# ksahlin/BESST

Hardware: AMD Instinct MI355X
Metric: read-pairs/sec into scaffold graph; edge-set match + gap MAE vs CPU ref (higher is better)
Workload: dtype int32/int64 (fp64 for read_len truncation); 1 GPU; C3: 100000 contigs / 200000000 read-pairs, one rf library with 22 % PE contamination, 400000000 records resident in HBM (1 copy cycled); records_per_gpu=400000000, edge_rows=263235, parallelism=single GPU, generator=besst_amd.synth.simulate_library_device (torch ops on the GPU, seeded), 1.5 s

## Files before the change

### besst_amd/csrc/classify.hip

```cpp
#include <stdarg.h>
#include <stdio.h>
#include <stdlib.h>

#include <atomic>
#include <type_traits>

#include "common.h"

namespace besst {

namespace {

constexpr uint32_t kNoSlot = 0xffffffffu;

constexpr uint32_t EV_COV = 1u, EV_FISHY = 2u, EV_NONUNIQ = 4u, EV_REACH = 8u,
                   EV_DOUBLE = 32u, EV_MAPQ0 = 64u, EV_CASEA = 128u, EV_FIRSTMIN = 256u;

enum : int { kSpecGeneric = 0, kSpecFr = 1, kSpecRf = 2 };

__device__ __forceinline__ uint32_t ins_thr_u32(const ClassifyArgs& a) {
    return a.ins_thr_int <= 0 ? 0u : (uint32_t)a.ins_thr_int;
}

struct Eval {
// ... 1299 lines not shown
        a.has_any = last_idx >= 0 ? 1 : 0;
        a.l1 = last_idx >= 0 ? s_l1[last_idx] : 0;
        a.l2 = last_idx >= 0 ? s_l2[last_idx] : 0;
        a.head_present = s_first[0] > 0 ? 1 : 0;
        a.f1 = s_first[1]; a.f2 = s_first[2]; a.head_info = (uint32_t)s_first[3];
        int tot = 0, tot_runs = 0;
        for (int w = 0; w < 16; ++w) { tot += s_sum[w]; tot_runs += s_sum_runs[w]; }
        a.total = (uint32_t)tot;
        a.runs = (uint32_t)tot_runs;
        agg[blockIdx.x] = a;
    }
}

template <bool kRuns>
__global__ __launch_bounds__(1024) void stitch_kernel(SummView summ, uint32_t nblocks, int32_t* carry, int detect,
                                                      uint32_t* __restrict__ offsets,
                                                      uint32_t* __restrict__ skip_slot,
                                                      uint32_t* n_out,
                                                      unsigned long long* counters,
                                                      const int32_t* __restrict__ tails, int rank,
                                                      int32_t* __restrict__ slice_info,
                                                      const StitchAgg* __restrict__ agg,
                                                      const int32_t* __restrict__ carry_in, uint32_t span,
                                                      uint32_t* __restrict__ run_offsets) {
    __shared__ int32_t s_l1[1024 * kStitchRounds], s_l2[1024 * kStitchRounds];
    __shared__ int s_any;
    __shared__ int s_head_block;
    __shared__ int32_t s_head[4];
    __shared__ int s_tab[64];
    __shared__ int s_total;
    using acc_t = typename std::conditional<kRuns, long long, int>::type;
    auto pack_counts = [](uint32_t tuples, uint32_t runs) -> acc_t {
        if (kRuns) return (acc_t)((long long)tuples | ((long long)runs << 32));
        return (acc_t)tuples;
    };
    __shared__ acc_t s_tab64[64];
    __shared__ acc_t s_total64;
    __shared__ int32_t s_carry[2];
    __shared__ acc_t s_base;
    __shared__ int s_redc[16][7];
    const int t = threadIdx.x, lane = t & 63, wave = t >> 6;
    const bool last_span = blockIdx.x == gridDim.x - 1;
    if (t == 0) {
        int32_t p1 = agg ? carry_in[0] : carry[0], p2 = agg ? carry_in[1] : carry[1];
        if (tails)
            for (int j = 0; j < rank; ++j)
                if (tails[j * 4]) { p1 = tails[j * 4 + 1]; p2 = tails[j * 4 + 2]; }
        int any = 0;
        acc_t base = 0;
        for (uint32_t j = 0; j < blockIdx.x; ++j) {
            const StitchAgg a = agg[j];
            acc_t tot = (acc_t)a.total;
            if (kRuns) tot = (acc_t)((long long)a.total | ((long long)a.runs << 32));
            if (a.head_present && !(slice_info && !any)) {
                const CEDelta d = create_edge(a.f1, a.f2, p1, p2, a.head_info & 1u, a.head_info & 2u, a.head_info & 4u,
                                              detect != 0);
                if ((a.head_info & 8u) && !d.keep) tot -= 1ll + (a.runs ? 1ll << 32 : 0ll);
            }
            base += tot;
            if (a.has_any) { p1 = a.l1; p2 = a.l2; any = 1; }
        }
        s_carry[0] = p1; s_carry[1] = p2; s_base = base;
        s_any = any; s_head_block = -1;
    }
    __syncthreads();
// ... 317 lines not shown
    __syncthreads();
    if (threadIdx.x == 0) {
        atomicAdd(&counts[0], (unsigned long long)(s_c[0] + s_c[1] + s_c[2] + s_c[3]));
        atomicAdd(&counts[1], (unsigned long long)(s_m[0] + s_m[1] + s_m[2] + s_m[3]));
    }
}

__global__ void resolve_carry_kernel(const int32_t* __restrict__ tails, int rank, int32_t* __restrict__ carry) {
    if (threadIdx.x != 0) return;
    for (int j = 0; j < rank; ++j)
        if (tails[j * 4]) { carry[0] = tails[j * 4 + 1]; carry[1] = tails[j * 4 + 2]; }
}

}

namespace {
std::atomic<int> g_last_form{-1};
}
int classify_last_form() { return g_last_form.load(); }

bool classify_can_group_runs(const ClassifyArgs& a) {
    static const int knob = [] { const char* e = getenv("BESST_LOOP_RUNS"); return e ? atoi(e) : 1; }();
    return knob != 0 && a.record_path == 1 && a.n > 0;
}

int launch_classify_scan(hipStream_t s, const ClassifyArgs& a, int64_t* aligned, besst_counters* counters,
                         void* ws, size_t ws_bytes, bool group_runs) {
    if (a.n <= 0) return BESST_OK;
    BESST_REQUIRE(a.n < (int64_t)1 << 32, "classify: more than 2^32-1 records in one call");
    const ClsWorkspace w = carve(ws, a.n);
    BESST_REQUIRE(ws != nullptr && ws_bytes >= w.total, "classify: workspace too small");
    const uint32_t nblocks = (uint32_t)((a.n + kClsTile - 1) / kClsTile);
    const uint32_t stream_blocks = (uint32_t)((a.n + kStreamTile - 1) / kStreamTile);
    BESST_REQUIRE(!group_runs || classify_can_group_runs(a), "classify: this record loop cannot group runs");
    if (a.record_path == 1) {
        if (group_runs) BESST_HIP_TRY(hipMemsetAsync(w.run_status, 0, 4, s));
        ProfScope ps(s, kProfFusedWave);
        auto* al = reinterpret_cast<unsigned long long*>(aligned);
        const bool side = a.cs_off && a.mate_bits && a.tid_bits;
        g_last_form.store(side ? 3 : a.mate_bits ? (a.tid_bits ? 2 : 1) : 0);
        if (side) {
            const uint32_t full = (uint32_t)(a.n / kClsTile);
            const char* const spec_env = getenv("BESST_LOOP_SPEC");
            const bool spec = !(spec_env && atoi(spec_env) == 0) && a.read_len_int >= 0 && a.extend_paths != 0 && a.no_score == 0 && a.detect_dup != 0;
            const int form = spec ? (a.rf != 0 ? kSpecRf : kSpecFr) : kSpecGeneric;
#define BESST_LAUNCH_LEAN(RUNS, SPEC)                                                                                   \
// ... 277 lines not shown
int launch_classify_emit(hipStream_t s, int64_t n, int detect_dup, int32_t* carry, uint64_t* keys,
                         uint64_t* payload, uint32_t* n_out, besst_counters* counters, void* ws,
                         size_t ws_bytes, const uint8_t* cls8, int32_t n_contigs, int64_t* aligned,
                         const int32_t* tails, int rank, int32_t* slice_info, PresortSpec* presort) {
    PresortSpec pre{};
    if (presort && presort->table) {
        pre = *presort;
        BESST_REQUIRE(pre.rows > 0 && (pre.rows & (pre.rows - 1)) == 0 && pre.shift >= 0 && pre.shift <= 47, "classify: bad presort description");
        if (!pre.in_record_loop) BESST_HIP_TRY(hipMemsetAsync(pre.table, 0, (size_t)pre.rows * 512 * sizeof(uint32_t), s));
    }
    if (n <= 0) {
        BESST_HIP_TRY(hipMemsetAsync(n_out, 0, sizeof(uint32_t), s));
        if (slice_info) BESST_HIP_TRY(hipMemsetAsync(slice_info, 0, 8 * sizeof(int32_t), s));
        if (presort) presort->segmented = 0;
        return BESST_OK;
    }
    const ClsWorkspace w = carve(ws, n);
    BESST_REQUIRE(ws != nullptr && ws_bytes >= w.total, "classify: workspace too small");
    const uint32_t nblocks = (uint32_t)((n + kClsTile - 1) / kClsTile);
    auto* ctr = reinterpret_cast<unsigned long long*>(counters);
    const bool grouped = pre.table && pre.in_record_loop == 3;
    BESST_REQUIRE(!grouped || (pre.segmented && !slice_info && !tails), "classify: grouped runs need the segmented hand-over");
    uint32_t* run_offsets = grouped ? w.run_offsets : nullptr;
    {
        ProfScope ps(s, kProfStitch);
        uint32_t span = kStitchSpan;
        if (const char* e = getenv("BESST_STITCH_SPAN")) {
            const long v = atol(e);
            if (v >= 1 && v < (long)kStitchSpan) span = (uint32_t)v;
        }
        const uint32_t spans = (nblocks + span - 1) / span;
        BESST_REQUIRE(spans <= w.agg_spans, "classify: too many stitch spans for the workspace");
        if (spans > 1) {
            int32_t* carry_in = reinterpret_cast<int32_t*>(w.agg + w.agg_spans);
            hipLaunchKernelGGL(stitch_spans_kernel, dim3(spans), dim3(1024), 0, s, w.summ, nblocks, span, detect_dup, carry,
                               w.agg, carry_in);
            if (run_offsets)
                hipLaunchKernelGGL(stitch_kernel<true>, dim3(spans), dim3(1024), 0, s, w.summ, nblocks, carry, detect_dup, w.offsets,
                                   w.skip, n_out, ctr, tails, rank, slice_info, w.agg, carry_in, span, run_offsets);
            else
                hipLaunchKernelGGL(stitch_kernel<false>, dim3(spans), dim3(1024), 0, s, w.summ, nblocks, carry, detect_dup, w.offsets,
                                   w.skip, n_out, ctr, tails, rank, slice_info, w.agg, carry_in, span, run_offsets);
        } else {
            if (run_offsets)
                hipLaunchKernelGGL(stitch_kernel<true>, dim3(1), dim3(1024), 0, s, w.summ, nblocks, carry, detect_dup, w.offsets,
                                   w.skip, n_out, ctr, tails, rank, slice_info, (const StitchAgg*)nullptr,
                                   (const int32_t*)nullptr, span, run_offsets);
            else
                hipLaunchKernelGGL(stitch_kernel<false>, dim3(1), dim3(1024), 0, s, w.summ, nblocks, carry, detect_dup, w.offsets,
                                   w.skip, n_out, ctr, tails, rank, slice_info, (const StitchAgg*)nullptr,
                                   (const int32_t*)nullptr, span, run_offsets);
        }
    }
    {
        PresortSpec in_compact = pre;
        const bool segmented = pre.table && pre.in_record_loop && pre.segmented && !slice_info && !tails;
        if (pre.table && pre.in_record_loop) {
            ProfScope ps(s, kProfFixup);
            hipLaunchKernelGGL(presort_fixup_kernel, dim3((nblocks + 255) / 256), dim3(256), 0, s, w.seg_keys, w.skip, nblocks, pre,
                               segmented ? cls8 : nullptr, n_contigs, reinterpret_cast<unsigned long long*>(aligned),
                               w.offsets, n_out, (segmented && !grouped) ? w.chunk_first : nullptr);
            in_compact.table = nullptr;
        }
        if (segmented) {
            presort->segmented = 1;
            presort->seg = SegSource{w.seg_keys, w.seg_payload, w.offsets, w.skip, nblocks, (uint32_t)kClsTile, payload, w.chunk_first,
                                     grouped ? w.run_offsets : nullptr, w.summ.p, w.summ.stride, w.run_status};
        } else {
            if (presort) presort->segmented = 0;
            ProfScope ps(s, kProfCompact);
            hipLaunchKernelGGL(compact_kernel, dim3(nblocks), dim3(256), 0, s, w.summ, w.offsets, w.skip, w.seg_keys,
                               w.seg_payload, keys, payload, cls8, n_contigs, reinterpret_cast<unsigned long long*>(aligned),
                               in_compact);
        }
    }
    BESST_HIP_TRY(hipGetLastError());
    return BESST_OK;
}

int launch_classify(hipStream_t s, const ClassifyArgs& a, int32_t* carry, int64_t* aligned, uint64_t* keys,
// ... 29 lines not shown
```

### besst_amd/csrc/common.h

```cpp
#pragma once

#include <hip/hip_runtime.h>
#include <stdint.h>

#include "../../include/besst_amd.h"
#include "bgzf_scan.h"

namespace besst {

void set_error(const char* fmt, ...);

#define BESST_HIP_TRY(expr)                                                                  \
    do {                                                                                     \
        hipError_t _e = (expr);                                                              \
        if (_e != hipSuccess) {                                                              \
            besst::set_error("%s failed: %s (%s:%d)", #expr, hipGetErrorString(_e), __FILE__, \
                             __LINE__);                                                      \
            return BESST_ERR_HIP;                                                            \
        }                                                                                    \
    } while (0)

#define BESST_REQUIRE(cond, msg)                 \
    do {                                         \
        if (!(cond)) {                           \
// ... 257 lines not shown
int launch_candidate_density(hipStream_t s, int64_t n, const int32_t* tid, const int32_t* mtid, int64_t sample_records,
                             unsigned long long* counts);
int launch_mate_bits(hipStream_t s, const int32_t* tid, const int32_t* mtid, int64_t lo, int64_t hi, int64_t n, uint8_t* bits,
                     uint8_t* tid_bits);
int launch_cand_offsets(hipStream_t s, int64_t n, int64_t n_refs, const int32_t* tid, const int32_t* mtid,
                        const uint16_t* flag, uint8_t* set_bits, uint32_t* offsets, uint8_t* mate_bits, uint8_t* tid_bits,
                        uint32_t first_block = 0);
int launch_cand_entries(hipStream_t s, int64_t n, const int32_t* tid, const int32_t* mtid, const int32_t* pos,
                        const int32_t* mpos, const uint16_t* flag, const uint8_t* mapq, const uint16_t* qlen,
                        const uint8_t* set_bits, const uint32_t* offsets, int32_t* e_tid, int32_t* e_mtid, int32_t* e_pos,
                        int32_t* e_mpos, uint32_t* e_fq, uint8_t* e_mapq, uint32_t cap,
                        uint32_t first_block = 0);
int classify_last_form();
int launch_classify_tail(hipStream_t s, int64_t n, int32_t* tail, void* ws, size_t ws_bytes);
int launch_resolve_carry(hipStream_t s, const int32_t* tails, int rank, int32_t* carry);
int launch_classify_emit(hipStream_t s, int64_t n, int detect_dup, int32_t* carry, uint64_t* keys,
                         uint64_t* payload, uint32_t* n_out, besst_counters* counters, void* ws,
                         size_t ws_bytes, const uint8_t* cls8, int32_t n_contigs, int64_t* aligned,
                         const int32_t* tails, int rank, int32_t* slice_info, PresortSpec* presort = nullptr);

size_t reduce_workspace_bytes(int64_t cap);
bool sort_presort_spec(int64_t cap, int key_bits, uint64_t key_base, void* ws, size_t ws_bytes, PresortSpec* out);
bool onesweep_presort_spec(int64_t cap, int key_bits, uint64_t key_base, void* ws, PresortSpec* out);
int launch_sort_reduce(hipStream_t s, int64_t cap, const uint32_t* n_tuples, int key_bits,
                       const uint64_t* keys, const uint64_t* payload, uint64_t* row_key,
                       uint32_t* row_mask, uint32_t* row_n, int64_t* row_sum, int64_t* row_sum_sq,
                       uint32_t* row_first, uint32_t* row_offset, int32_t* obs_lo, int32_t* obs_hi,
                       uint32_t* n_rows, void* ws, size_t ws_bytes, const uint32_t* first_map = nullptr,
                       uint64_t key_base = 0, bool hist_ready = false, const SegSource* seg = nullptr,
                       uint32_t flags = 0 );
bool runs_enabled(int64_t cap);
size_t runs_workspace_bytes(int64_t cap);
int launch_runs_reduce(hipStream_t s, int64_t cap, const uint32_t* n_tuples, int key_bits, const uint64_t* keys,
                       const uint64_t* payload, const SegSource* seg, uint64_t* grouped, void* staged_rows,
                       uint64_t* row_key, uint32_t* row_mask, uint32_t* row_n, int64_t* row_sum, int64_t* row_sum_sq,
                       uint32_t* row_first, uint32_t* row_offset, int32_t* obs_lo, int32_t* obs_hi, uint32_t* n_rows,
                       void* ws, size_t ws_bytes, const uint32_t* first_map, uint64_t key_base);
void* onesweep_staged_rows(void* ws, int64_t cap);
int reduce_census(hipStream_t s, int64_t cap, int key_bits, uint32_t flags, const void* ws, size_t ws_bytes, int64_t* out);
bool onesweep_takes_bucket_form(int64_t cap, int key_bits);
int onesweep_census(int64_t cap, const void* ws, int64_t* counts );
size_t onesweep_workspace_bytes(int64_t cap);
int launch_onesweep_sort_reduce(hipStream_t s, int64_t cap, const uint32_t* n_tuples, int key_bits,
                                const uint64_t* keys, const uint64_t* payload, uint64_t* buf_keys[2],
                                uint32_t* buf_idx[2], uint64_t* row_key, uint32_t* row_mask, uint32_t* row_n,
                                int64_t* row_sum, int64_t* row_sum_sq, uint32_t* row_first, uint32_t* row_offset,
                                int32_t* obs_lo, int32_t* obs_hi, uint32_t* n_rows, void* ws, size_t ws_bytes,
                                const uint32_t* first_map, uint64_t key_base, bool hist_ready = false,
                                const SegSource* seg = nullptr);
size_t exchange_region_bytes(int64_t pair_cap);
size_t exchange_stride_bytes(int64_t pair_cap, int64_t rider_bytes);
int launch_partition(hipStream_t s, int64_t cap, const uint32_t* n_tuples, int node_bits, int world,
                     const uint64_t* keys, const uint64_t* payload, int64_t pair_cap, void* send, void* ws,
// ... 69 lines not shown
```

### besst_amd/csrc/runs.hip

```cpp
#include "common.h"

namespace besst {

namespace {

constexpr int kRgRounds = BESST_RG_ROUNDS;
constexpr int kRgMinWaves = kRgRounds >= 16 ? 3 : kRgRounds >= 8 ? 5 : 8;
constexpr int kRgChunk = 64 * kRgRounds;
static_assert(kRgChunk == kRunChunk, "the record loop's chunk table is cut for this chunk size");
constexpr int kRgWaves = 4;
constexpr int kRgPeel = 63;
constexpr uint32_t kRgNoSlot = 0xffffffffu;
constexpr int kRgCopyRuns = 8;
constexpr int kRsThreads = 256, kRsItems = 16, kRsTile = kRsThreads * kRsItems;

struct RunRec {
    uint64_t key;
    unsigned long long sum, sq;
    uint32_t n, first, off, mask;
};
static_assert(sizeof(RunRec) == 40, "run record layout");

__device__ __forceinline__ uint64_t rg_readlane64(uint64_t v, int l) {
    return ((uint64_t)(uint32_t)__builtin_amdgcn_readlane((int)(v >> 32), l) << 32) |
// ... 313 lines not shown
    }
#pragma unroll
    for (int d = 32; d > 0; d >>= 1) before += (uint32_t)__shfl_xor((int)before, d, 64);
    if (lane == 63) s_w[wave] = x;
    if (lane == 0) s_b[wave] = before;
    __syncthreads();
    uint32_t off = x - tot;
#pragma unroll
    for (int q = 0; q < kRsThreads / 64; ++q) {
        if (q < wave) off += s_w[q];
        off += s_b[q];
    }
#pragma unroll
    for (int q = 0; q < kRsItems; ++q) {
        const uint32_t j = j0 + (uint32_t)(t * kRsItems + q);
        if (j < n) {
            run_dst[j] = off;
            if (dst_of) dst_of[(uint32_t)run_at[j]] = off;
        }
        off += len[q];
    }
}

__global__ __launch_bounds__(256) void rg_rows_kernel(const uint32_t* __restrict__ status, uint32_t* __restrict__ n_rows,
                                                      const uint32_t* __restrict__ r_runs, const uint32_t* __restrict__ r_first_run,
                                                      const int32_t* __restrict__ run_at, const uint32_t* __restrict__ run_dst,
                                                      const RunRec* __restrict__ staged, uint32_t* __restrict__ row_mask,
                                                      uint32_t* __restrict__ row_n, unsigned long long* __restrict__ row_sum,
                                                      unsigned long long* __restrict__ row_sum_sq,
                                                      uint32_t* __restrict__ row_first, uint32_t* __restrict__ row_offset) {
    const uint32_t st_err = status[0], st_over = status[1];
    if (st_err | st_over) {
        if (blockIdx.x == 0 && threadIdx.x == 0) *n_rows = st_err ? BESST_ROWS_SORT_FAILED : BESST_ROWS_RUN_OVERFLOW;
        return;
    }
    const uint32_t r = blockIdx.x * blockDim.x + threadIdx.x;
    const uint32_t nr = *n_rows;
    if (nr >= BESST_ROWS_RUN_OVERFLOW || r >= nr) return;
    const uint32_t j0 = r_first_run[r], c = r_runs[r];
    uint32_t nn = 0, first = 0, mask = 0;
    unsigned long long s = 0, q = 0;
    for (uint32_t j = j0; j < j0 + c; ++j) {
        const RunRec rec = staged[(uint32_t)run_at[j]];
        nn += rec.n;
        s += rec.sum;
        q += rec.sq;
// ... 143 lines not shown
    k.hdr[1] = (uint32_t)(lane + 64) < k.nch ? h1 : 0ull;
    uint32_t before = 0;
#pragma unroll
    for (int q = 0; q < 2; ++q) {
        const uint32_t n = (uint32_t)(k.hdr[q] >> 32) & 0xffffu;
        uint32_t x = n;
#pragma unroll
        for (int d = 1; d < 64; d <<= 1) {
            const uint32_t v = (uint32_t)__shfl_up((int)x, d, 64);
            if (lane >= d) x += v;
        }
        k.ex[q] = before + x - n;
        before += (uint32_t)__builtin_amdgcn_readlane((int)x, 63);
    }
    k.total = before;
    return k;
}
static_assert(kRlMaxChunks <= 64, "rl_list_kernel searches the chunk prefixes one wave holds");
constexpr int kRlWaves = 4;
constexpr int kRlSingletonRuns = 32;

__global__ __launch_bounds__(256) void rl_list_kernel(SegSource seg, uint32_t run_cap, uint64_t* __restrict__ run_keys,
                                                      uint64_t* __restrict__ run_payload, RunCols rc,
                                                      uint32_t* __restrict__ n_runs, uint32_t* __restrict__ status) {
    const int lane = threadIdx.x & 63;
    const uint32_t b = blockIdx.x * 4u + (uint32_t)__builtin_amdgcn_readfirstlane((int)(threadIdx.x >> 6));
    if (b >= seg.nblocks) return;
    const char* region0 = reinterpret_cast<const char*>(seg.seg_keys + (size_t)b * seg.tile);
    uint64_t key = reinterpret_cast<const uint64_t*>(region0 + kRlKeys)[lane];
    uint32_t meta = reinterpret_cast<const uint32_t*>(region0 + kRlMeta)[lane];
    const RlBlock k = rl_block(seg, b, lane);
    if (k.head_kept && lane == 0 && k.head_idx < run_cap) {
        run_keys[k.head_idx] = *reinterpret_cast<const uint64_t*>(k.region + kRlHeadKey);
        run_payload[k.head_idx] = 1ull | ((uint64_t)k.head_idx << 32);
        rc.first[k.head_idx] = k.off + k.hslot;
        rc.mask[k.head_idx] = (uint32_t)(k.pl_p[k.hslot] >> 62);
    }
    if (b == seg.nblocks - 1u && lane == 0) {
        const uint32_t all = k.run0 + k.total;
        if (all > run_cap || *seg.run_status != 0u) {
            status[1] = 1u;
            status[2] = all;
            *n_runs = 0u;
        } else {
            *n_runs = all;
        }
    }
    for (uint32_t r0 = 0; r0 < k.total; r0 += 64u) {
        const uint32_t r = r0 + (uint32_t)lane;
        uint32_t c = 0;
#pragma unroll
        for (int step = 32; step > 0; step >>= 1) {
            const uint32_t t = c + (uint32_t)step;
            const uint32_t ex_t = (uint32_t)__shfl((int)k.ex[0], (int)(t & 63u), 64);
            if (t < k.nch && ex_t <= r) c = t;
        }
        const uint32_t ex_c = (uint32_t)__shfl((int)k.ex[0], (int)c, 64);
        const uint32_t lo = (uint32_t)__shfl((int)(uint32_t)k.hdr[0], (int)c, 64);
        const uint32_t e = c * (uint32_t)kRlSlots + (r - ex_c);
        if (r < k.total) {
            if (!(r0 == 0u && c == 0u)) {
                key = reinterpret_cast<const uint64_t*>(k.region + kRlKeys)[e];
// ... 155 lines not shown

}

constexpr int64_t kRunCapMax = (int64_t)4 << 20;

static int64_t rg_run_cap(int64_t cap) { return cap < kRunCapMax ? cap : kRunCapMax; }

static RgWorkspace rg_carve(void* ws, int64_t cap) {
    RgWorkspace w;
    char* p = static_cast<char*>(ws);
    size_t off = 0;
    const size_t rc = (size_t)rg_run_cap(cap);
    const size_t nchunks = align_up((size_t)((cap + kRgChunk - 1) / kRgChunk), kRgWaves);
    w.run_cap = (uint32_t)rc;
    w.status = reinterpret_cast<uint32_t*>(p + off); off += 256;
    w.n_runs = w.status + 8;
    w.chunk_runs = reinterpret_cast<uint32_t*>(p + off); off += align_up(nchunks * 4, 256);
    w.starts = reinterpret_cast<uint16_t*>(p + off); off += align_up((size_t)cap * 2, 256);
    w.run_keys = reinterpret_cast<uint64_t*>(p + off); off += align_up(rc * 8, 256);
    w.run_payload = reinterpret_cast<uint64_t*>(p + off); off += align_up(rc * 8, 256);
    w.run_len = reinterpret_cast<int32_t*>(p + off); off += align_up(rc * 4, 256);
    w.run_at = reinterpret_cast<int32_t*>(p + off); off += align_up(rc * 4, 256);
    w.run_dst = reinterpret_cast<uint32_t*>(p + off); off += align_up(rc * 4, 256);
    w.tile_sum = reinterpret_cast<uint32_t*>(p + off); off += align_up(((rc + kRsTile - 1) / kRsTile) * 4, 256);
    w.r_mask = reinterpret_cast<uint32_t*>(p + off); off += align_up(rc * 4, 256);
    w.r_runs = reinterpret_cast<uint32_t*>(p + off); off += align_up(rc * 4, 256);
    w.r_sum = reinterpret_cast<int64_t*>(p + off); off += align_up(rc * 8, 256);
    w.r_sq = reinterpret_cast<int64_t*>(p + off); off += align_up(rc * 8, 256);
    w.r_first = reinterpret_cast<uint32_t*>(p + off); off += align_up(rc * 4, 256);
    w.r_first_run = reinterpret_cast<uint32_t*>(p + off); off += align_up(rc * 4, 256);
    w.nested = p + off;
    w.nested_bytes = reduce_workspace_bytes((int64_t)rc);
    off += align_up(w.nested_bytes, 256);
    w.total = off;
    return w;
}

size_t runs_workspace_bytes(int64_t cap) {
    if (cap < 1) cap = 1;
    return rg_carve(nullptr, cap).total;
}

bool runs_enabled(int64_t cap) {
    return cap >= 1 && cap <= ((int64_t)1 << 30);
}

int launch_runs_reduce(hipStream_t s, int64_t cap, const uint32_t* n_tuples, int key_bits, const uint64_t* keys,
                       const uint64_t* payload, const SegSource* seg, uint64_t* grouped, void* staged_rows,
                       uint64_t* row_key, uint32_t* row_mask, uint32_t* row_n, int64_t* row_sum, int64_t* row_sum_sq,
                       uint32_t* row_first, uint32_t* row_offset, int32_t* obs_lo, int32_t* obs_hi, uint32_t* n_rows,
                       void* ws, size_t ws_bytes, const uint32_t* first_map, uint64_t key_base) {
    const RgWorkspace w = rg_carve(ws, cap);
    BESST_REQUIRE(ws != nullptr && ws_bytes >= w.total, "reduce: run workspace too small");
    BESST_REQUIRE(grouped != nullptr && staged_rows != nullptr, "reduce: run buffers missing");
    RunRec* staged = static_cast<RunRec*>(staged_rows);
    const uint32_t nchunks = (uint32_t)((cap + kRgChunk - 1) / kRgChunk);
    const uint32_t grid1 = (nchunks + kRgWaves - 1) / kRgWaves;
    BESST_HIP_TRY(hipMemsetAsync(w.status, 0, 64, s));
    if (seg && seg->run_offsets) {
        BESST_REQUIRE(!first_map && seg->summ && seg->run_status, "reduce: incomplete description of the record loop's runs");
        RunCols rc;
        {
            char* p = static_cast<char*>(staged_rows);
            const size_t n = (size_t)w.run_cap;
            rc.sum = reinterpret_cast<unsigned long long*>(p); p += n * 8;
            rc.sq = reinterpret_cast<unsigned long long*>(p); p += n * 8;
            rc.first = reinterpret_cast<uint32_t*>(p); p += n * 4;
            rc.mask = reinterpret_cast<uint32_t*>(p); p += n * 4;
            rc.dst = reinterpret_cast<uint32_t*>(p);
        }
        const uint32_t bgrid = seg->nblocks;
        {
            ProfScope ps(s, kProfRunList);
            hipLaunchKernelGGL(rl_list_kernel, dim3((bgrid + 3u) / 4u), dim3(256), 0, s, *seg, w.run_cap, w.run_keys, w.run_payload, rc,
                               w.n_runs, w.status);
        }
        const int rcode = launch_sort_reduce(s, (int64_t)w.run_cap, w.n_runs, key_bits, w.run_keys, w.run_payload, row_key, w.r_mask,
                                             w.r_runs, w.r_sum, w.r_sq, w.r_first, w.r_first_run, w.run_len, w.run_at, n_rows,
                                             w.nested, w.nested_bytes, nullptr, key_base, false, nullptr, BESST_REDUCE_NO_RUNS);
        if (rcode) return rcode;
        const uint32_t tiles = (w.run_cap + kRsTile - 1) / kRsTile;
        {
            ProfScope ps(s, kProfRunScan);
            hipLaunchKernelGGL(rg_tile_sums_kernel, dim3(tiles), dim3(kRsThreads), 0, s, w.run_len, w.n_runs, w.tile_sum);
            hipLaunchKernelGGL(rg_dst_kernel, dim3(tiles), dim3(kRsThreads), 0, s, w.run_len, w.n_runs, w.tile_sum, w.run_dst,
                               w.run_at, rc.dst);
        }
        {
            ProfScope ps(s, kProfRunPlace);
            hipLaunchKernelGGL(rl_place_kernel, dim3(bgrid), dim3(kRlWaves * 64), 0, s, *seg, w.status, n_rows, rc, obs_lo, obs_hi);
        }
        {
            ProfScope ps(s, kProfRunRows);
            hipLaunchKernelGGL(rl_rows_kernel, dim3((w.run_cap + 255) / 256), dim3(256), 0, s, w.status, n_rows, w.r_runs,
                               w.r_first_run, w.run_len, w.run_at, w.run_dst, rc.first, rc.mask, rc.sum, rc.sq, row_mask, row_n,
                               reinterpret_cast<unsigned long long*>(row_sum), reinterpret_cast<unsigned long long*>(row_sum_sq),
                               row_first, row_offset);
        }
        BESST_HIP_TRY(hipGetLastError());
        return BESST_OK;
    }
    {
        ProfScope ps(s, kProfRunGroup);
        if (seg)
            hipLaunchKernelGGL((rg_group_kernel<true>), dim3(grid1), dim3(kRgWaves * 64), 0, s, keys, payload, *seg, n_tuples,
                               (uint32_t)cap, first_map, grouped, staged, w.starts, w.chunk_runs);
        else
            hipLaunchKernelGGL((rg_group_kernel<false>), dim3(grid1), dim3(kRgWaves * 64), 0, s, keys, payload, SegSource{},
                               n_tuples, (uint32_t)cap, first_map, grouped, staged, w.starts, w.chunk_runs);
// ... 34 lines not shown
```

### besst_amd/csrc/sortreduce.hip

```cpp
#include <unistd.h>

#include <atomic>
#include <random>
#include <type_traits>
#include <vector>

#include "common.h"

namespace besst {

namespace {

__device__ __forceinline__ uint32_t nblocks_of(uint32_t n, uint32_t tile) { return (n + tile - 1) / tile; }

__device__ __forceinline__ uint32_t digit_of(uint64_t key, const DigitSel& ds) {
    if (ds.mode == 0) return (uint32_t)((key - ds.base) >> ds.shift) & ((1u << ds.bits) - 1u);
    const uint32_t scaf = (uint32_t)(key >> (2 + ds.node_bits));
    return owner_of_scaffold(scaf, ds.world);
}

#ifndef BESST_SCAN_FREE_MAX_BLOCKS
#define BESST_SCAN_FREE_MAX_BLOCKS 64
#endif
constexpr int kScanFreeMaxBlocks = BESST_SCAN_FREE_MAX_BLOCKS;
// ... 595 lines not shown
        bitonic_pairs(gk, gx, np);
        for (int i = threadIdx.x; i < n; i += blockDim.x) {
            keys[s0 + i] = gk[i];
            if (!kPacked) idx[s0 + i] = gx[i];
            if (kPacked) heads += (i == 0 || (gk[i] >> packed_bits) != (gk[i - 1] >> packed_bits)) ? 1u : 0u;
        }
    }
    if (kPacked) {
#pragma unroll
        for (int d = 32; d > 0; d >>= 1) heads += (uint32_t)__shfl_xor((int)heads, d, 64);
        if ((threadIdx.x & 63) == 0 && heads) atomicAdd(&s_heads, heads);
        __syncthreads();
        if (threadIdx.x == 0) bucket_rows[blockIdx.x] = s_heads;
    }
}

__global__ __launch_bounds__(256) void bucket_reduce_kernel(
    const uint64_t* __restrict__ words, const uint64_t* __restrict__ payload, const uint32_t* __restrict__ n_ptr,
    const uint32_t* __restrict__ bucket_start, const uint32_t* __restrict__ bucket_rows, int packed_bits, int msd_shift,
    uint32_t* __restrict__ n_rows, uint64_t* __restrict__ row_key, uint32_t* __restrict__ row_mask,
    uint32_t* __restrict__ row_n, unsigned long long* __restrict__ row_sum,
    unsigned long long* __restrict__ row_sum_sq, uint32_t* __restrict__ row_first, uint32_t* __restrict__ row_offset,
    int32_t* __restrict__ obs_lo, int32_t* __restrict__ obs_hi, const uint32_t* __restrict__ first_map,
    uint64_t key_base, const unsigned long long* __restrict__ msd_flags, unsigned long long nonce) {
    __shared__ uint32_t s_part[4];
    __shared__ int s_wheads[4];
    const int t = threadIdx.x, lane = t & 63, wave = t >> 6;
    const uint32_t b = blockIdx.x;
    const uint32_t n_all = *n_ptr;
    const uint32_t s0 = bucket_start[b], e0 = bucket_start[b + 1];
    if (msd_flags && msd_flags[1] == nonce) {
        if (b == 0 && t == 0) *n_rows = BESST_ROWS_SORT_FAILED;
        return;
    }
    if (n_all == 0) {
        if (b == 0 && t == 0) *n_rows = 0;
        return;
    }
    uint32_t pre = 0;
    for (uint32_t bb = t; bb < b; bb += 256) pre += bucket_rows[bb];
#pragma unroll
    for (int d = 32; d > 0; d >>= 1) pre += (uint32_t)__shfl_xor((int)pre, d, 64);
    if (lane == 0) s_part[wave] = pre;
    __syncthreads();
    const uint32_t base = s_part[0] + s_part[1] + s_part[2] + s_part[3];
    if (b == gridDim.x - 1 && t == 0) *n_rows = base + bucket_rows[b];
    const int n = (int)(e0 - s0);
    if (n == 0) return;
    const uint64_t idx_mask = (1ull << packed_bits) - 1ull;
    const unsigned long long le_mask = lane == 63 ? ~0ull : ((2ull << lane) - 1ull);
    int64_t rows_done = (int64_t)base;
    for (int c0 = 0; c0 < n; c0 += 256) {
        const int j = c0 + t;
        const bool live = j < n;
        const uint32_t i = s0 + (uint32_t)j;
        const uint64_t w = live ? words[i] : ~0ull;
        const uint64_t key = ((uint64_t)b << msd_shift) | (w >> packed_bits);
        const uint32_t src = (uint32_t)(w & idx_mask);
        const uint64_t pkey = (live && j > 0) ? (((uint64_t)b << msd_shift) | (words[i - 1] >> packed_bits)) : ~key;
        const bool head = live && (j == 0 || key != pkey);
        const unsigned long long hmask = __ballot(head);
        if (lane == 0) s_wheads[wave] = __popcll(hmask);
        __syncthreads();
        int wpre = 0, ctot = 0;
#pragma unroll
        for (int q = 0; q < 4; ++q) {
            if (q < wave) wpre += s_wheads[q];
            ctot += s_wheads[q];
        }
        const int64_t row = rows_done + wpre + __popcll(hmask & le_mask) - 1;
        uint64_t pl = 0;
        if (live) pl = payload[src];
        const uint32_t lo = (uint32_t)pl, hi = (uint32_t)(pl >> 32);
        const int32_t o_lo = (int32_t)lo, o_hi = (int32_t)(hi & 0x3fffffffu);
        if (live) {
            obs_lo[i] = o_lo;
            obs_hi[i] = o_hi;
            if (head) {
                row_key[row] = key + key_base;
                row_mask[row] = hi >> 30;
                row_first[row] = first_map ? first_map[src] : src;
                row_offset[row] = i;
            }
        }
        {
            const unsigned long long starts = hmask | 1ull;
            const int start = 63 - __clzll((long long)(starts & le_mask));
            uint32_t cn = live ? 1u : 0u;
            unsigned long long cs = live ? (unsigned long long)((long long)o_lo + o_hi) : 0ull;
            unsigned long long cq = cs * cs;
#pragma unroll
            for (int d = 1; d < 64; d <<= 1) {
                const uint32_t on = (uint32_t)__shfl_up((int)cn, d, 64);
                const unsigned long long os = __shfl_up(cs, d, 64), oq = __shfl_up(cq, d, 64);
                if (lane - d >= start) { cn += on; cs += os; cq += oq; }
            }
            const unsigned long long lmask = __ballot(live);
            const bool tail = live && (lane == 63 || !((lmask >> (lane + 1)) & 1ull) || ((hmask >> (lane + 1)) & 1ull));
            if (tail) {
                atomicAdd(&row_n[row], cn);
                atomicAdd(&row_sum[row], cs);
                atomicAdd(&row_sum_sq[row], cq);
            }
        }
        rows_done += ctot;
        __syncthreads();
    }
}

constexpr int kRowScanFreeMaxBlocks = 2048;

__global__ __launch_bounds__(kRedThreads) void row_heads_kernel(const uint64_t* __restrict__ keys,
                                                                const uint32_t* __restrict__ n_ptr, uint32_t cap,
                                                                uint32_t* __restrict__ blk_heads, int packed_bits) {
    __shared__ int s_w[4];
    const int t = threadIdx.x, lane = t & 63, wave = t >> 6;
    const uint32_t b = blockIdx.x;
    const uint32_t i0 = b * kRedTile + t * kRedItems;
    uint64_t k[kRedItems + 1];
    k[0] = (i0 > 0 && i0 - 1 < cap) ? keys[i0 - 1] >> packed_bits : 0ull;
#pragma unroll
    for (int j = 0; j < kRedItems; ++j) k[j + 1] = (i0 + j) < cap ? keys[i0 + j] >> packed_bits : 0ull;
    uint32_t n = *n_ptr;
    n = n < cap ? n : cap;
    if (b >= nblocks_of(n, kRedTile)) return;
    int cnt = 0;
#pragma unroll
    for (int j = 0; j < kRedItems; ++j) {
        const uint32_t i = i0 + j;
// ... 297 lines not shown

static bool bucket_words_packable(int64_t cap, int key_bits) {
    return (key_bits > kMsdBits ? key_bits - kMsdBits : 0) + index_bits(cap) <= 64;
}

static bool takes_large_stream_path(int64_t cap, int key_bits) {
    const uint32_t nb_sort = (uint32_t)((cap + kSortTile - 1) / kSortTile);
    return !(nb_sort <= (uint32_t)kScanFreeMaxBlocks ||
             (bucket_words_packable(cap, key_bits) && nb_sort <= (uint32_t)kMsdMaxBlocks));
}

bool sort_presort_spec(int64_t cap, int key_bits, uint64_t key_base, void* ws, size_t ws_bytes, PresortSpec* out) {
    if (!out || !ws || cap < 1 || cap >= ((int64_t)1 << 32) || key_bits < 1 || key_bits > 64) return false;
    const RedWorkspace w = carve(ws, cap);
    if (ws_bytes < w.total || !takes_large_stream_path(cap, key_bits)) return false;
    return onesweep_presort_spec(cap, key_bits, key_base, w.os_ws, out);
}

int launch_sort_reduce(hipStream_t s, int64_t cap, const uint32_t* n_tuples, int key_bits,
                       const uint64_t* keys, const uint64_t* payload, uint64_t* row_key,
                       uint32_t* row_mask, uint32_t* row_n, int64_t* row_sum, int64_t* row_sum_sq,
                       uint32_t* row_first, uint32_t* row_offset, int32_t* obs_lo, int32_t* obs_hi,
                       uint32_t* n_rows, void* ws, size_t ws_bytes, const uint32_t* first_map, uint64_t key_base,
                       bool hist_ready, const SegSource* seg, uint32_t flags) {
    BESST_REQUIRE(cap >= 0 && cap < ((int64_t)1 << 32), "reduce: capacity out of range");
    BESST_REQUIRE(key_bits >= 1 && key_bits <= 64, "reduce: key_bits out of range");
    if (cap == 0) {
        BESST_HIP_TRY(hipMemsetAsync(n_rows, 0, sizeof(uint32_t), s));
        return BESST_OK;
    }
    const RedWorkspace w = carve(ws, cap);
    BESST_REQUIRE(ws != nullptr && ws_bytes >= w.total, "reduce: workspace too small");
    BESST_REQUIRE(!seg || takes_large_stream_path(cap, key_bits), "reduce: a segmented stream needs the large-stream sort");
    const uint32_t nb_sort = (uint32_t)((cap + kSortTile - 1) / kSortTile);
    const uint32_t nb_red = (uint32_t)((cap + kRedTile - 1) / kRedTile);
    auto* zsum = reinterpret_cast<unsigned long long*>(row_sum);
    auto* zsq = reinterpret_cast<unsigned long long*>(row_sum_sq);
    const uint64_t* kin = keys;
    const uint32_t* iin = nullptr;
    int packed_bits = 0;
    const int cap_idx_bits = index_bits(cap);
    const bool packable = bucket_words_packable(cap, key_bits);
    if (!takes_large_stream_path(cap, key_bits)) {
        const int shift = key_bits > kMsdBits ? key_bits - kMsdBits : 0;
        const DigitSel ds{0, shift, 0, 1u, kMsdBits, key_base};
        packed_bits = packable ? cap_idx_bits : 0;
        const bool one_launch = packed_bits != 0 && msd_one_launch() != 0 && nb_sort <= (uint32_t)kMsdMaxBlocks;
// ... 10 lines not shown
                hipLaunchKernelGGL((msd_partition_kernel<kMsdItems, true>), dim3(2u * nb_part), dim3(kSortThreads), 0, s, keys,
                                   n_tuples, (uint32_t)cap, ds, w.row_total, w.msd_flags, nonce, msd_spin_limit(), w.keys[0],
                                   w.bucket_start, packed_bits, row_n, zsum, zsq, w.table);
        } else if (nb_sort <= (uint32_t)kMsdSmallMaxBlocks) {
            const uint32_t nb_small = (uint32_t)((cap + kSortThreads * kMsdSmallItems - 1) / (kSortThreads * kMsdSmallItems));
            launch_pass<kMsdBits, kMsdSmallItems>(s, w, nb_small, (uint32_t)cap, n_tuples, ds, true, keys, nullptr,
                                                  w.keys[0], w.idx[0], row_n, zsum, zsq, w.bucket_start, packed_bits);
        } else {
            launch_pass<kMsdBits>(s, w, nb_sort, (uint32_t)cap, n_tuples, ds, true, keys, nullptr, w.keys[0], w.idx[0],
                                  row_n, zsum, zsq, w.bucket_start, packed_bits);
        }
        if (shift > 0 || packed_bits) {
            ProfScope ps(s, kProfBucketSort);
            const dim3 grid(1u << kMsdBits), block(kBucketThreads);
            if (!packed_bits)
                hipLaunchKernelGGL((bucket_sort_kernel<false, kBucketLds>), grid, block, 0, s, w.keys[0], w.idx[0],
                                   w.bucket_start, n_tuples, w.big_keys, w.big_idx, w.bucket_rows, 0, shift, mflags, nonce);
            else
                hipLaunchKernelGGL((bucket_sort_kernel<true, kBucketPackedCap>), grid, block, 0, s, w.keys[0], w.idx[0],
                                   w.bucket_start, n_tuples, w.big_keys, w.big_idx, w.bucket_rows, packed_bits, shift, mflags, nonce);
        }
        if (packed_bits) {
            ProfScope ps(s, kProfBucketReduce);
            hipLaunchKernelGGL(bucket_reduce_kernel, dim3(1u << kMsdBits), dim3(256), 0, s, w.keys[0], payload, n_tuples,
                               w.bucket_start, w.bucket_rows, packed_bits, shift, n_rows, row_key, row_mask, row_n, zsum, zsq,
                               row_first, row_offset, obs_lo, obs_hi, first_map, key_base, mflags, nonce);
            BESST_HIP_TRY(hipGetLastError());
            return BESST_OK;
        }
        kin = w.keys[0];
        iin = w.idx[0];
    } else {
        if (w.rg_bytes && !(flags & BESST_REDUCE_NO_RUNS))
            return launch_runs_reduce(s, cap, n_tuples, key_bits, keys, payload, seg, seg ? seg->payload_out : w.keys[0],
                                      onesweep_staged_rows(w.os_ws, cap), row_key, row_mask, row_n, row_sum, row_sum_sq,
                                      row_first, row_offset, obs_lo, obs_hi, n_rows, w.rg_ws, w.rg_bytes, first_map, key_base);
        uint64_t* bk[2] = {w.keys[0], w.keys[1]};
        uint32_t* bi[2] = {w.idx[0], w.idx[1]};
        return launch_onesweep_sort_reduce(s, cap, n_tuples, key_bits, keys, payload, bk, bi, row_key, row_mask, row_n,
                                           row_sum, row_sum_sq, row_first, row_offset, obs_lo, obs_hi, n_rows, w.os_ws,
                                           w.os_bytes, first_map, key_base, hist_ready, seg);
    }
    const int rscanned = nb_red > (uint32_t)kRowScanFreeMaxBlocks ? 1 : 0;
    {
        ProfScope ps(s, kProfRowHeads);
        hipLaunchKernelGGL(row_heads_kernel, dim3(nb_red), dim3(kRedThreads), 0, s, kin, n_tuples, (uint32_t)cap,
                           w.blk_heads, packed_bits);
    }
    if (rscanned) {
// ... 320 lines not shown
```

Baseline: 192.1 billion read-pairs/s.

## Fold fixup, status clear and run-length tile sums into neighbouring kernels

The stitch kernel now zeroes aligned counts for contigs with class 0, which replaces the separate presort fixup launch on the grouped path. The run-list kernel clears the status words itself instead of issuing a memset. The bucket reduce kernel accumulates per-bucket run-length sums, so a single bucket-indexed prefix kernel can replace the two-pass tile-sum and dst scan. The goal is fewer kernel launches and fewer passes over memory, at the cost of extra work in the stitch kernel and serial per-block prefix loops over buckets.

```diff
diff --git a/besst_amd/csrc/classify.hip b/besst_amd/csrc/classify.hip
--- a/besst_amd/csrc/classify.hip
+++ b/besst_amd/csrc/classify.hip
@@ -1345,7 +1345,9 @@
                                                       int32_t* __restrict__ slice_info,
                                                       const StitchAgg* __restrict__ agg,
                                                       const int32_t* __restrict__ carry_in, uint32_t span,
-                                                      uint32_t* __restrict__ run_offsets) {
+                                                      uint32_t* __restrict__ run_offsets,
+                                                      const uint8_t* __restrict__ cls8, int32_t n_contigs,
+                                                      unsigned long long* __restrict__ aligned) {
     __shared__ int32_t s_l1[1024 * kStitchRounds], s_l2[1024 * kStitchRounds];
     __shared__ int s_any;
     __shared__ int s_head_block;
@@ -1364,6 +1366,19 @@
     __shared__ int s_redc[16][7];
     const int t = threadIdx.x, lane = t & 63, wave = t >> 6;
     const bool last_span = blockIdx.x == gridDim.x - 1;
+    if (kRuns && cls8) {
+        const uint32_t nc = (uint32_t)n_contigs, gt = blockIdx.x * blockDim.x + (uint32_t)t, nt = gridDim.x * blockDim.x;
+        const uint32_t n16 = (reinterpret_cast<uintptr_t>(cls8) & 15u) == 0 ? nc / 16u : 0u;
+        for (uint32_t g = gt; g < n16; g += nt) {
+            const uint4 v = reinterpret_cast<const uint4*>(cls8)[g];
+            const uint32_t w4[4] = {v.x, v.y, v.z, v.w};
+#pragma unroll
+            for (int k = 0; k < 16; ++k)
+                if (((w4[k >> 2] >> (8 * (k & 3))) & 255u) == 0u) aligned[g * 16u + (uint32_t)k] = 0;
+        }
+        for (uint32_t c = n16 * 16u + gt; c < nc; c += nt)
+            if (!cls8[c]) aligned[c] = 0;
+    }
     if (t == 0) {
         int32_t p1 = agg ? carry_in[0] : carry[0], p2 = agg ? carry_in[1] : carry[1];
         if (tails)
@@ -1727,6 +1742,15 @@
 bool classify_can_group_runs(const ClassifyArgs& a) {
     static const int knob = [] { const char* e = getenv("BESST_LOOP_RUNS"); return e ? atoi(e) : 1; }();
     return knob != 0 && a.record_path == 1 && a.n > 0;
+}
+
+namespace {
+
+bool env_on(const char* name) {
+    const char* const e = getenv(name);
+    return !(e && atoi(e) == 0);
+}
+
 }
 
 int launch_classify_scan(hipStream_t s, const ClassifyArgs& a, int64_t* aligned, besst_counters* counters,
@@ -2050,6 +2074,9 @@
     const bool grouped = pre.table && pre.in_record_loop == 3;
     BESST_REQUIRE(!grouped || (pre.segmented && !slice_info && !tails), "classify: grouped runs need the segmented hand-over");
     uint32_t* run_offsets = grouped ? w.run_offsets : nullptr;
+    const bool fixup_in_stitch = grouped && !pre.count && cls8 && env_on("BESST_STITCH_FIXUP");
+    const uint8_t* const zero_cls8 = fixup_in_stitch ? cls8 : nullptr;
+    auto* al = reinterpret_cast<unsigned long long*>(aligned);
     {
         ProfScope ps(s, kProfStitch);
         uint32_t span = kStitchSpan;
@@ -2065,25 +2092,27 @@
                                w.agg, carry_in);
             if (run_offsets)
                 hipLaunchKernelGGL(stitch_kernel<true>, dim3(spans), dim3(1024), 0, s, w.summ, nblocks, carry, detect_dup, w.offsets,
-                                   w.skip, n_out, ctr, tails, rank, slice_info, w.agg, carry_in, span, run_offsets);
+                                   w.skip, n_out, ctr, tails, rank, slice_info, w.agg, carry_in, span, run_offsets, zero_cls8, n_contigs, al);
             else
                 hipLaunchKernelGGL(stitch_kernel<false>, dim3(spans), dim3(1024), 0, s, w.summ, nblocks, carry, detect_dup, w.offsets,
-                                   w.skip, n_out, ctr, tails, rank, slice_info, w.agg, carry_in, span, run_offsets);
+                                   w.skip, n_out, ctr, tails, rank, slice_info, w.agg, carry_in, span, run_offsets, zero_cls8, n_contigs, al);
         } else {
             if (run_offsets)
                 hipLaunchKernelGGL(stitch_kernel<true>, dim3(1), dim3(1024), 0, s, w.summ, nblocks, carry, detect_dup, w.offsets,
                                    w.skip, n_out, ctr, tails, rank, slice_info, (const StitchAgg*)nullptr,
-                                   (const int32_t*)nullptr, span, run_offsets);
+                                   (const int32_t*)nullptr, span, run_offsets, zero_cls8, n_contigs, al);
             else
                 hipLaunchKernelGGL(stitch_kernel<false>, dim3(1), dim3(1024), 0, s, w.summ, nblocks, carry, detect_dup, w.offsets,
                                    w.skip, n_out, ctr, tails, rank, slice_info, (const StitchAgg*)nullptr,
-                                   (const int32_t*)nullptr, span, run_offsets);
+                                   (const int32_t*)nullptr, span, run_offsets, zero_cls8, n_contigs, al);
         }
     }
     {
         PresortSpec in_compact = pre;
         const bool segmented = pre.table && pre.in_record_loop && pre.segmented && !slice_info && !tails;
-        if (pre.table && pre.in_record_loop) {
+        if (pre.table && pre.in_record_loop && fixup_in_stitch) {
+            in_compact.table = nullptr;
+        } else if (pre.table && pre.in_record_loop) {
             ProfScope ps(s, kProfFixup);
             hipLaunchKernelGGL(presort_fixup_kernel, dim3((nblocks + 255) / 256), dim3(256), 0, s, w.seg_keys, w.skip, nblocks, pre,
                                segmented ? cls8 : nullptr, n_contigs, reinterpret_cast<unsigned long long*>(aligned),
diff --git a/besst_amd/csrc/common.h b/besst_amd/csrc/common.h
--- a/besst_amd/csrc/common.h
+++ b/besst_amd/csrc/common.h
@@ -303,13 +303,19 @@
 size_t reduce_workspace_bytes(int64_t cap);
 bool sort_presort_spec(int64_t cap, int key_bits, uint64_t key_base, void* ws, size_t ws_bytes, PresortSpec* out);
 bool onesweep_presort_spec(int64_t cap, int key_bits, uint64_t key_base, void* ws, PresortSpec* out);
+constexpr int kBucketSumWords = 2048;
+struct BucketSums {
+    uint32_t* len_sum;
+    const uint32_t* bucket_start;
+    uint32_t buckets;
+};
 int launch_sort_reduce(hipStream_t s, int64_t cap, const uint32_t* n_tuples, int key_bits,
                        const uint64_t* keys, const uint64_t* payload, uint64_t* row_key,
                        uint32_t* row_mask, uint32_t* row_n, int64_t* row_sum, int64_t* row_sum_sq,
                        uint32_t* row_first, uint32_t* row_offset, int32_t* obs_lo, int32_t* obs_hi,
                        uint32_t* n_rows, void* ws, size_t ws_bytes, const uint32_t* first_map = nullptr,
                        uint64_t key_base = 0, bool hist_ready = false, const SegSource* seg = nullptr,
-                       uint32_t flags = 0 );
+                       uint32_t flags = 0 , BucketSums* bucket_sums = nullptr);
 bool runs_enabled(int64_t cap);
 size_t runs_workspace_bytes(int64_t cap);
 int launch_runs_reduce(hipStream_t s, int64_t cap, const uint32_t* n_tuples, int key_bits, const uint64_t* keys,
diff --git a/besst_amd/csrc/runs.hip b/besst_amd/csrc/runs.hip
--- a/besst_amd/csrc/runs.hip
+++ b/besst_amd/csrc/runs.hip
@@ -359,6 +359,56 @@
     }
 }
 
+__global__ __launch_bounds__(256) void rg_dst_bucket_kernel(const int32_t* __restrict__ run_len,
+                                                            const uint32_t* __restrict__ n_runs,
+                                                            const uint32_t* __restrict__ n_rows,
+                                                            const uint32_t* __restrict__ bucket_start,
+                                                            const uint32_t* __restrict__ len_sum,
+                                                            uint32_t* __restrict__ run_dst,
+                                                            const int32_t* __restrict__ run_at,
+                                                            uint32_t* __restrict__ dst_of) {
+    __shared__ uint32_t s_w[4], s_b[4];
+    const int t = threadIdx.x, lane = t & 63, wave = t >> 6;
+    const uint32_t b = blockIdx.x;
+    const uint32_t n = *n_runs;
+    if (n == 0u || *n_rows >= BESST_ROWS_RUN_OVERFLOW) return;
+    uint32_t s0 = bucket_start[b], e0 = bucket_start[b + 1];
+    s0 = s0 < n ? s0 : n;
+    e0 = e0 < n ? e0 : n;
+    if (e0 <= s0) return;
+    uint32_t before = 0;
+    for (uint32_t bb = t; bb < b; bb += 256) before += len_sum[bb];
+#pragma unroll
+    for (int d = 32; d > 0; d >>= 1) before += (uint32_t)__shfl_xor((int)before, d, 64);
+    if (lane == 0) s_b[wave] = before;
+    __syncthreads();
+    uint32_t base = s_b[0] + s_b[1] + s_b[2] + s_b[3];
+    for (uint32_t j0 = s0; j0 < e0; j0 += 256u) {
+        const uint32_t j = j0 + (uint32_t)t;
+        const uint32_t len = j < e0 ? (uint32_t)run_len[j] : 0u;
+        uint32_t x = len;
+#pragma unroll
+        for (int d = 1; d < 64; d <<= 1) {
+            const uint32_t v = (uint32_t)__shfl_up((int)x, d, 64);
+            if (lane >= d) x += v;
+        }
+        if (lane == 63) s_w[wave] = x;
+        __syncthreads();
+        uint32_t off = base + x - len, tot = 0;
+#pragma unroll
+        for (int q = 0; q < 4; ++q) {
+            if (q < wave) off += s_w[q];
+            tot += s_w[q];
+        }
+        if (j < e0) {
+            run_dst[j] = off;
+            if (dst_of) dst_of[(uint32_t)run_at[j]] = off;
+        }
+        base += tot;
+        __syncthreads();
+    }
+}
+
 __global__ __launch_bounds__(256) void rg_rows_kernel(const uint32_t* __restrict__ status, uint32_t* __restrict__ n_rows,
                                                       const uint32_t* __restrict__ r_runs, const uint32_t* __restrict__ r_first_run,
                                                       const int32_t* __restrict__ run_at, const uint32_t* __restrict__ run_dst,
@@ -548,7 +598,7 @@
 
 __global__ __launch_bounds__(256) void rl_list_kernel(SegSource seg, uint32_t run_cap, uint64_t* __restrict__ run_keys,
                                                       uint64_t* __restrict__ run_payload, RunCols rc,
-                                                      uint32_t* __restrict__ n_runs, uint32_t* __restrict__ status) {
+                                                      uint32_t* n_runs, uint32_t* status, int clear_status) {
     const int lane = threadIdx.x & 63;
     const uint32_t b = blockIdx.x * 4u + (uint32_t)__builtin_amdgcn_readfirstlane((int)(threadIdx.x >> 6));
     if (b >= seg.nblocks) return;
@@ -564,6 +614,9 @@
     }
     if (b == seg.nblocks - 1u && lane == 0) {
         const uint32_t all = k.run0 + k.total;
+        if (clear_status)
+            for (int q = 0; q < 16; ++q)
+                if (status + q != n_runs) status[q] = 0u;
         if (all > run_cap || *seg.run_status != 0u) {
             status[1] = 1u;
             status[2] = all;
@@ -765,7 +818,8 @@
     w.run_len = reinterpret_cast<int32_t*>(p + off); off += align_up(rc * 4, 256);
     w.run_at = reinterpret_cast<int32_t*>(p + off); off += align_up(rc * 4, 256);
     w.run_dst = reinterpret_cast<uint32_t*>(p + off); off += align_up(rc * 4, 256);
-    w.tile_sum = reinterpret_cast<uint32_t*>(p + off); off += align_up(((rc + kRsTile - 1) / kRsTile) * 4, 256);
+    const size_t sums = (rc + kRsTile - 1) / kRsTile;
+    w.tile_sum = reinterpret_cast<uint32_t*>(p + off); off += align_up((sums > (size_t)kBucketSumWords ? sums : (size_t)kBucketSumWords) * 4, 256);
     w.r_mask = reinterpret_cast<uint32_t*>(p + off); off += align_up(rc * 4, 256);
     w.r_runs = reinterpret_cast<uint32_t*>(p + off); off += align_up(rc * 4, 256);
     w.r_sum = reinterpret_cast<int64_t*>(p + off); off += align_up(rc * 8, 256);
@@ -799,7 +853,9 @@
     RunRec* staged = static_cast<RunRec*>(staged_rows);
     const uint32_t nchunks = (uint32_t)((cap + kRgChunk - 1) / kRgChunk);
     const uint32_t grid1 = (nchunks + kRgWaves - 1) / kRgWaves;
-    BESST_HIP_TRY(hipMemsetAsync(w.status, 0, 64, s));
+    const char* const ls_env = getenv("BESST_LIST_STATUS");
+    const bool list_clears = seg && seg->run_offsets && seg->nblocks > 0 && !(ls_env && atoi(ls_env) == 0);
+    if (!list_clears) BESST_HIP_TRY(hipMemsetAsync(w.status, 0, 64, s));
     if (seg && seg->run_offsets) {
         BESST_REQUIRE(!first_map && seg->summ && seg->run_status, "reduce: incomplete description of the record loop's runs");
         RunCols rc;
@@ -816,18 +872,26 @@
         {
             ProfScope ps(s, kProfRunList);
             hipLaunchKernelGGL(rl_list_kernel, dim3((bgrid + 3u) / 4u), dim3(256), 0, s, *seg, w.run_cap, w.run_keys, w.run_payload, rc,
-                               w.n_runs, w.status);
-        }
+                               w.n_runs, w.status, list_clears ? 1 : 0);
+        }
+        const char* const bs_env = getenv("BESST_BUCKET_SCAN");
+        BucketSums bsums{(bs_env && atoi(bs_env) == 0) ? nullptr : w.tile_sum, nullptr, 0u};
         const int rcode = launch_sort_reduce(s, (int64_t)w.run_cap, w.n_runs, key_bits, w.run_keys, w.run_payload, row_key, w.r_mask,
                                              w.r_runs, w.r_sum, w.r_sq, w.r_first, w.r_first_run, w.run_len, w.run_at, n_rows,
-                                             w.nested, w.nested_bytes, nullptr, key_base, false, nullptr, BESST_REDUCE_NO_RUNS);
+                                             w.nested, w.nested_bytes, nullptr, key_base, false, nullptr, BESST_REDUCE_NO_RUNS,
+                                             &bsums);
         if (rcode) return rcode;
         const uint32_t tiles = (w.run_cap + kRsTile - 1) / kRsTile;
         {
             ProfScope ps(s, kProfRunScan);
-            hipLaunchKernelGGL(rg_tile_sums_kernel, dim3(tiles), dim3(kRsThreads), 0, s, w.run_len, w.n_runs, w.tile_sum);
-            hipLaunchKernelGGL(rg_dst_kernel, dim3(tiles), dim3(kRsThreads), 0, s, w.run_len, w.n_runs, w.tile_sum, w.run_dst,
-                               w.run_at, rc.dst);
+            if (bsums.buckets) {
+                hipLaunchKernelGGL(rg_dst_bucket_kernel, dim3(bsums.buckets), dim3(256), 0, s, w.run_len, w.n_runs, n_rows,
+                                   bsums.bucket_start, w.tile_sum, w.run_dst, w.run_at, rc.dst);
+            } else {
+                hipLaunchKernelGGL(rg_tile_sums_kernel, dim3(tiles), dim3(kRsThreads), 0, s, w.run_len, w.n_runs, w.tile_sum);
+                hipLaunchKernelGGL(rg_dst_kernel, dim3(tiles), dim3(kRsThreads), 0, s, w.run_len, w.n_runs, w.tile_sum, w.run_dst,
+                                   w.run_at, rc.dst);
+            }
         }
         {
             ProfScope ps(s, kProfRunPlace);
diff --git a/besst_amd/csrc/sortreduce.hip b/besst_amd/csrc/sortreduce.hip
--- a/besst_amd/csrc/sortreduce.hip
+++ b/besst_amd/csrc/sortreduce.hip
@@ -641,8 +641,10 @@
     uint32_t* __restrict__ row_n, unsigned long long* __restrict__ row_sum,
     unsigned long long* __restrict__ row_sum_sq, uint32_t* __restrict__ row_first, uint32_t* __restrict__ row_offset,
     int32_t* __restrict__ obs_lo, int32_t* __restrict__ obs_hi, const uint32_t* __restrict__ first_map,
-    uint64_t key_base, const unsigned long long* __restrict__ msd_flags, unsigned long long nonce) {
+    uint64_t key_base, const unsigned long long* __restrict__ msd_flags, unsigned long long nonce,
+    uint32_t* __restrict__ len_sum) {
     __shared__ uint32_t s_part[4];
+    __shared__ uint32_t s_len[4];
     __shared__ int s_wheads[4];
     const int t = threadIdx.x, lane = t & 63, wave = t >> 6;
     const uint32_t b = blockIdx.x;
@@ -665,7 +667,11 @@
     const uint32_t base = s_part[0] + s_part[1] + s_part[2] + s_part[3];
     if (b == gridDim.x - 1 && t == 0) *n_rows = base + bucket_rows[b];
     const int n = (int)(e0 - s0);
-    if (n == 0) return;
+    if (n == 0) {
+        if (len_sum && t == 0) len_sum[b] = 0u;
+        return;
+    }
+    uint32_t len_acc = 0;
     const uint64_t idx_mask = (1ull << packed_bits) - 1ull;
     const unsigned long long le_mask = lane == 63 ? ~0ull : ((2ull << lane) - 1ull);
     int64_t rows_done = (int64_t)base;
@@ -695,6 +701,7 @@
         if (live) {
             obs_lo[i] = o_lo;
             obs_hi[i] = o_hi;
+            len_acc += lo;
             if (head) {
                 row_key[row] = key + key_base;
                 row_mask[row] = hi >> 30;
@@ -724,6 +731,13 @@
         }
         rows_done += ctot;
         __syncthreads();
+    }
+    if (len_sum) {
+#pragma unroll
+        for (int d = 32; d > 0; d >>= 1) len_acc += (uint32_t)__shfl_xor((int)len_acc, d, 64);
+        if (lane == 0) s_len[wave] = len_acc;
+        __syncthreads();
+        if (t == 0) len_sum[b] = s_len[0] + s_len[1] + s_len[2] + s_len[3];
     }
 }
 
@@ -1067,7 +1081,8 @@
                        uint32_t* row_mask, uint32_t* row_n, int64_t* row_sum, int64_t* row_sum_sq,
                        uint32_t* row_first, uint32_t* row_offset, int32_t* obs_lo, int32_t* obs_hi,
                        uint32_t* n_rows, void* ws, size_t ws_bytes, const uint32_t* first_map, uint64_t key_base,
-                       bool hist_ready, const SegSource* seg, uint32_t flags) {
+                       bool hist_ready, const SegSource* seg, uint32_t flags, BucketSums* bucket_sums) {
+    if (bucket_sums) { bucket_sums->bucket_start = nullptr; bucket_sums->buckets = 0; }
     BESST_REQUIRE(cap >= 0 && cap < ((int64_t)1 << 32), "reduce: capacity out of range");
     BESST_REQUIRE(key_bits >= 1 && key_bits <= 64, "reduce: key_bits out of range");
     if (cap == 0) {
@@ -1124,9 +1139,15 @@
         }
         if (packed_bits) {
             ProfScope ps(s, kProfBucketReduce);
+            uint32_t* len_sum = nullptr;
+            if (bucket_sums && bucket_sums->len_sum && (1 << kMsdBits) <= kBucketSumWords) {
+                len_sum = bucket_sums->len_sum;
+                bucket_sums->bucket_start = w.bucket_start;
+                bucket_sums->buckets = 1u << kMsdBits;
+            }
             hipLaunchKernelGGL(bucket_reduce_kernel, dim3(1u << kMsdBits), dim3(256), 0, s, w.keys[0], payload, n_tuples,
                                w.bucket_start, w.bucket_rows, packed_bits, shift, n_rows, row_key, row_mask, row_n, zsum, zsq,
-                               row_first, row_offset, obs_lo, obs_hi, first_map, key_base, mflags, nonce);
+                               row_first, row_offset, obs_lo, obs_hi, first_map, key_base, mflags, nonce, len_sum);
             BESST_HIP_TRY(hipGetLastError());
             return BESST_OK;
         }
```

Result: no change. 193.3 billion read-pairs/s, median of 6 (+0.6%).
